# creare-com/pydem

Hardware: AMD Instinct MI355X
Metric: Mcells/s (slope+aspect+UCA+TWI end-to-end) per tile; % HBM roofline (higher is better)
Workload: dtype f64

## Files before the change

### pydem_amd/csrc/pits.hip

```cpp
#include "internal.h"
#include <hipcub/hipcub.hpp>
#include <math.h>
#include <stdlib.h>
#include <algorithm>
#include <vector>

namespace {

__device__ __forceinline__ double np_pairwise_leaf(const double *a, int n)
{
    if (n < 8) {
        double res = 0.;
        for (int i = 0; i < n; i++) res += a[i];
        return res;
    }
    double r0 = a[0], r1 = a[1], r2 = a[2], r3 = a[3], r4 = a[4], r5 = a[5], r6 = a[6], r7 = a[7];
    int i;
    for (i = 8; i < n - (n % 8); i += 8) {
        r0 += a[i]; r1 += a[i + 1]; r2 += a[i + 2]; r3 += a[i + 3];
        r4 += a[i + 4]; r5 += a[i + 5]; r6 += a[i + 6]; r7 += a[i + 7];
    }
    double res = ((r0 + r1) + (r2 + r3)) + ((r4 + r5) + (r6 + r7));
    for (; i < n; i++) res += a[i];
    return res;
// ... 392 lines not shown
        if (gl == 0) {
            if (P.overflow_list && flag[0] == 2) P.overflow_list[atomicAdd(P.overflow_count, 1)] = pit;
            else atomicAdd(&P.out_count[3], 1);
        }
        return;
    }
    if (ndrain < 0) { if (gl == 0) atomicAdd(&P.out_count[1], 1); return; }
    if (gl == 0) finish_pit(P, pit, ipit, jpit, epit, ndrain, dlist, dxy, sv, chunk_base, chunk_left, stk);

}

#ifndef PYDEM_WV_OCC
#define PYDEM_WV_OCC 6
#endif
#ifndef PYDEM_WV_CAP
#define PYDEM_WV_CAP 256
#endif
constexpr int WV_MAXD = 64;
constexpr int LN_W16 = 16;

template <int WW, int CAP, typename PosT>
struct WaveLds {
    static constexpr PosT HOLE = (PosT)~(PosT)0;
    static constexpr PosT PITBIT = (PosT)((PosT)1 << (sizeof(PosT) * 8 - 2));
    uint32_t seen[WW * WW / 32];
    double le[CAP];
    PosT lpos[CAP];
    uint16_t holes[CAP];
    union {
        PosT pq[CAP];
        struct { int32_t dl[WV_MAXD]; double dxy[WV_MAXD], sv[WV_MAXD]; } fin;
    } u;
};

__device__ __forceinline__ double min_f64(double a, double b)
{
    double r;
    asm("v_min_f64 %0, %1, %2" : "=v"(r) : "v"(a), "v"(b));
    return r;
}

template <int CTRL>
__device__ __forceinline__ double dpp_fmin(double v)
{
    const int lo = __double2loint(v), hi = __double2hiint(v);
    const int lo2 = __builtin_amdgcn_update_dpp(0, lo, CTRL, 0xF, 0xF, true);
    const int hi2 = __builtin_amdgcn_update_dpp(0, hi, CTRL, 0xF, 0xF, true);
    return min_f64(v, __hiloint2double(hi2, lo2));
}
#if defined(__HIP_DEVICE_COMPILE__) && !defined(__gfx950__)
#error "wave_min uses the gfx9 DPP row broadcasts (row_bcast:15 / row_bcast:31, removed in gfx10+): this library is built for gfx950 only"
#endif
__device__ __forceinline__ double wave_min(double v)
{
    v = dpp_fmin<0xB1>(v);
    v = dpp_fmin<0x4E>(v);
    v = dpp_fmin<0x141>(v);
    v = dpp_fmin<0x140>(v);
    v = dpp_fmin<0x142>(v);
    v = dpp_fmin<0x143>(v);
    const int lo = __double2loint(v), hi = __double2hiint(v);
    return __hiloint2double(__builtin_amdgcn_readlane(hi, 63), __builtin_amdgcn_readlane(lo, 63));
}
__device__ __forceinline__ void wave_sync()
{
    __builtin_amdgcn_fence(__ATOMIC_SEQ_CST, "wavefront");
    __builtin_amdgcn_wave_barrier();
}

template <int W2, int W2_CAP, typename PosT>
__device__ void solve_pit_wave(const PitParams &P, int32_t pit, int lane, WaveLds<W2, W2_CAP, PosT> &L, int32_t &chunk_base,
                               int32_t &chunk_left, const uint32_t *state = nullptr)
{
    constexpr int W2_SLOTS = W2_CAP / 64;
    constexpr PosT W2_HOLE = WaveLds<W2, W2_CAP, PosT>::HOLE, W2_PITBIT = WaveLds<W2, W2_CAP, PosT>::PITBIT;
    const int n = P.n, m = P.m;
    const int ipit = pit / m, jpit = pit - ipit * m;
    const unsigned long long lt = (1ull << lane) - 1ull;
    int r0 = ipit - W2 / 2, c0 = jpit - W2 / 2;
    if (r0 > n - W2) r0 = n - W2;
    if (c0 > m - W2) c0 = m - W2;
    if (r0 < 0) r0 = 0;
    if (c0 < 0) c0 = 0;
    for (int w = lane; w < W2 * W2 / 32; w += 64) L.seen[w] = 0;
    const double epit = P.elev[pit];
    double epit_border = epit;
    int nb = 0, nh = 0, n_alive = 0;
    bool has_np = false, has_p = false, has_nan = false;
    int over = 0;
    auto expand = [&](int nq) {
        for (int base = 0; base < nq * 8; base += 64) {
            const int idx = base + lane;
            bool isnew = false, out = false;
            double e = 0.0; uint32_t pm = 0; int npos = 0;
            if (idx < nq * 8) {
                const int pos = L.u.pq[idx >> 3], d = idx & 7;
                const int di = d < 3 ? -1 : (d < 5 ? 0 : 1);
                const int dj = d < 3 ? d - 1 : (d == 3 ? -1 : (d == 4 ? 1 : d - 6));
                const int r = pos / W2, c = pos % W2;
                const int ii = r0 + r + di, jj = c0 + c + dj;
                if (ii >= 0 && ii < n && jj >= 0 && jj < m) {
                    const int rr = r + di, cc = c + dj;
                    if (rr < 0 || rr >= W2 || cc < 0 || cc >= W2) out = true;
                    else {
                        npos = rr * W2 + cc;
                        const uint32_t bit = 1u << (npos & 31);
                        const uint32_t old = atomicOr(&L.seen[npos >> 5], bit);
                        if (!(old & bit)) {
                            isnew = true;
                            const int64_t cell = (int64_t)ii * m + jj;
                            e = P.elev[cell]; pm = P.pitmask[cell];
                        }
                    }
                }
            }
            if (__ballot(out)) over = 1;
            const unsigned long long bal = __ballot(isnew);
            const int cnt = __popcll(bal);
            const int fresh = cnt > nh ? cnt - nh : 0;
            if (nb + fresh > W2_CAP) { over = 2; break; }
            if (isnew) {
                const int rk = __popcll(bal & lt);
                const int k = rk < nh ? (int)L.holes[nh - 1 - rk] : nb + (rk - nh);
                L.le[k] = e; L.lpos[k] = (PosT)((PosT)npos | (pm ? W2_PITBIT : (PosT)0));
            }
            if (__ballot(isnew && pm && e < epit)) has_p = true;
            if (__ballot(isnew && !pm && e < epit_border)) has_np = true;
            if (__ballot(isnew && e != e)) has_nan = true;
            nh -= cnt - fresh; nb += fresh; n_alive += cnt;
        }
        wave_sync();
    };
    int it0 = 0, nq0 = 1;
    if (state) {
        it0 = (int)state[0];
        epit_border = __hiloint2double((int)state[3], (int)state[2]);
        int lr0 = ipit - LN_W16 / 2, lc0 = jpit - LN_W16 / 2;
        if (lr0 > n - LN_W16) lr0 = n - LN_W16;
        if (lc0 > m - LN_W16) lc0 = m - LN_W16;
        if (lr0 < 0) lr0 = 0;
        if (lc0 < 0) lc0 = 0;
        const int dpos = (lr0 - r0) * W2 + (lc0 - c0);
        nq0 = 0;
#pragma unroll 1
        for (int j = 0; j < 4; j++) {
            const int cidx = lane + 64 * j;
            const bool in = (state[4 + 2 * j + (lane >> 5)] >> (lane & 31)) & 1u;
            const unsigned long long bal = __ballot(in);
            if (in) {
                const int pos = dpos + (cidx >> 4) * W2 + (cidx & 15);
                atomicOr(&L.seen[pos >> 5], 1u << (pos & 31));
                L.u.pq[nq0 + __popcll(bal & lt)] = (PosT)pos;
            }
            nq0 += __popcll(bal);
        }
    } else if (lane == 0) {
        const int pos = (ipit - r0) * W2 + (jpit - c0);
        L.seen[pos >> 5] = 1u << (pos & 31);
        L.u.pq[0] = (PosT)pos;
    }
    wave_sync();
    expand(nq0);
    if (!state && P.min_border) {
        double mn = INFINITY;
        for (int k = lane; k < nb; k += 64) mn = min_f64(mn, L.le[k]);
        mn = wave_min(mn);
        if (nb) epit_border = mn;
        has_np = false;
    }
    int mode = 0, ndrain = -1, it_used = it0;
    for (int it = it0; it < P.max_iter; it++) {
        if (over) break;
        if (n_alive == 0) break;
        if (has_nan) { if (has_p) mode = 2; break; }
        if (has_np) { mode = 1; break; }
        if (has_p) { mode = 2; break; }
        it_used = it + 1;
        double e[W2_SLOTS];
        double mn = INFINITY;
#pragma unroll
        for (int j = 0; j < W2_SLOTS; j++) {
            const int k = lane + 64 * j;
            e[j] = INFINITY;
            if (j * 64 < nb) {
                if (k < nb) e[j] = L.le[k];
                mn = min_f64(mn, e[j]);
            }
        }
        mn = wave_min(mn);
        int nq = 0;
#pragma unroll
        for (int j = 0; j < W2_SLOTS; j++) {
            if (j * 64 >= nb) break;
            const int k = lane + 64 * j;
            bool match = k < nb && e[j] == mn;
            PosT ps = 0;
            if (match) { ps = L.lpos[k]; match = ps != W2_HOLE; }
            const unsigned long long bal = __ballot(match);
            if (!bal) continue;
            if (match) {
                const int r = nq + __popcll(bal & lt);
                L.u.pq[r] = (PosT)(ps & (PosT)(W2_PITBIT - 1));
                L.holes[nh + r] = (uint16_t)k;
                L.le[k] = INFINITY; L.lpos[k] = W2_HOLE;
            }
            nq += __popcll(bal);
        }
        nh += nq; n_alive -= nq;
        wave_sync();
        expand(nq);
    }
    if (!over && mode) {
        int nd = 0;
        for (int base = 0; base < nb; base += 64) {
            const int k = base + lane;
            bool pred = false;
            int32_t cell = 0;
            if (k < nb && L.lpos[k] != W2_HOLE) {
                const int pos = (int)(L.lpos[k] & (PosT)(W2_PITBIT - 1));
                const bool pm = (L.lpos[k] & W2_PITBIT) != 0;
                const double ev = L.le[k];
                pred = mode == 1 ? (!pm && ev < epit_border) : (pm && ev < epit);
                cell = (int32_t)((int64_t)(r0 + pos / W2) * m + (c0 + pos % W2));
            }
            const unsigned long long bal = __ballot(pred);
            const int rank = nd + __popcll(bal & lt);
            wave_sync();
            if (pred && rank < WV_MAXD) L.u.fin.dl[rank] = cell;
            nd += __popcll(bal);
        }
        if (nd > WV_MAXD) over = 3;
        else {
            wave_sync();
            const int32_t key = lane < nd ? L.u.fin.dl[lane] : INT32_MAX;
            int rank = 0;
            for (int t = 0; t < nd; t++) rank += L.u.fin.dl[t] < key;
            wave_sync();
            if (lane < nd) L.u.fin.dl[rank] = key;
            wave_sync();
            ndrain = nd;
        }
    }
    if (lane == 0 && P.dbg) {
        const int idx = atomicAdd(&P.out_count[6], 1);
        P.dbg[4 * idx] = it_used; P.dbg[4 * idx + 1] = n_alive; P.dbg[4 * idx + 2] = over; P.dbg[4 * idx + 3] = ndrain;
    }
    if (over) {
        if (lane == 0) P.overflow_list[atomicAdd(P.overflow_count, 1)] = pit;
        return;
    }
    if (ndrain < 0) { if (lane == 0) atomicAdd(&P.out_count[1], 1); return; }
    finish_pit_wave(P, pit, ipit, jpit, epit, ndrain, L.u.fin.dl, L.u.fin.dxy, L.u.fin.sv, chunk_base, chunk_left, lane);
}

#include "pits_row.inl"

constexpr int LN_W = 16;
static_assert(LN_W == LN_W16, "hand-over records");
#ifndef PYDEM_LN_B
#define PYDEM_LN_B 32
#endif
constexpr int LN_B = PYDEM_LN_B;
#ifndef PYDEM_LN_T
#define PYDEM_LN_T 64
#endif
constexpr int LN_T = PYDEM_LN_T;

__device__ __forceinline__ double np_pairwise_leaf_strided(const double *a, int stride, int n)
{
    if (n < 8) {
        double res = 0.;
        for (int i = 0; i < n; i++) res += a[i * stride];
        return res;
    }
    double r0 = a[0], r1 = a[stride], r2 = a[2 * stride], r3 = a[3 * stride], r4 = a[4 * stride], r5 = a[5 * stride],
           r6 = a[6 * stride], r7 = a[7 * stride];
    int i;
    for (i = 8; i < n - (n % 8); i += 8) {
        r0 += a[i * stride]; r1 += a[(i + 1) * stride]; r2 += a[(i + 2) * stride]; r3 += a[(i + 3) * stride];
        r4 += a[(i + 4) * stride]; r5 += a[(i + 5) * stride]; r6 += a[(i + 6) * stride]; r7 += a[(i + 7) * stride];
    }
    double res = ((r0 + r1) + (r2 + r3)) + ((r4 + r5) + (r6 + r7));
    for (; i < n; i++) res += a[i * stride];
    return res;
}

__device__ __forceinline__ double np_pairwise_leaf15(const double *__restrict__ a, int n)
{
    double v[15];
#pragma unroll
    for (int k = 0; k < 15; k++) v[k] = a[k < n ? k : (n > 0 ? n - 1 : 0)];
    if (n < 8) {
        double res = 0.;
#pragma unroll
        for (int k = 0; k < 7; k++) if (k < n) res += v[k];
        return res;
    }
    double res = ((v[0] + v[1]) + (v[2] + v[3])) + ((v[4] + v[5]) + (v[6] + v[7]));
#pragma unroll
    for (int k = 8; k < 15; k++) if (k < n) res += v[k];
    return res;
}

constexpr int LN_CHUNK = 256;
constexpr int LN_FIN_BATCH = 32;

__global__ __launch_bounds__(LN_T) void k_pits_lane(PitParams P, const int32_t *__restrict__ pits, const int32_t *npits)
{
    __shared__ double s_e[LN_B * LN_T];
    __shared__ uint8_t s_p[LN_B * LN_T];
    __shared__ uint8_t s_q[LN_B * LN_T];
    __shared__ uint32_t s_seen[8 * LN_T];
    const int tid = threadIdx.x, lane = tid & 63;
    const unsigned long long lt = (1ull << lane) - 1ull;
    const int n = P.n, m = P.m;
    const int32_t np = *npits;
    double *const le = s_e + tid;
    uint8_t *const lp = s_p + tid, *const lq = s_q + tid;
    uint32_t *const seen = s_seen + tid;
    bool running = false, over = false, has_np = false, has_p = false, has_nan = false;
    int pending = 0;
    int32_t pit = 0;
    int r0 = 0, c0 = 0, ipit = 0, jpit = 0, nb = 0, it = 0;
    uint32_t pitbits = 0;
    double epit = 0.0, epit_border = 0.0;
    int32_t chunk_next = 0, chunk_end = 0;
    bool more = true;
    auto discover = [&](int r, int c) {
        const int wa = (r > 0 ? r - 1 : 0) >> 1, wb = (r < LN_W - 1 ? r + 1 : LN_W - 1) >> 1;
        uint32_t va = seen[wa * LN_T], vb = seen[wb * LN_T];
        if (wb == wa) vb = va;
#pragma unroll
        for (int k = 0; k < 8; k++) {
            const int di = k < 3 ? -1 : (k < 5 ? 0 : 1);
            const int dj = k < 3 ? k - 1 : (k == 3 ? -1 : (k == 4 ? 1 : k - 6));
            const int ii = r0 + r + di, jj = c0 + c + dj;
            const int rr = r + di, cc = c + dj;
            if (ii < 0 || ii >= n || jj < 0 || jj >= m) continue;
            if (rr < 0 || rr >= LN_W || cc < 0 || cc >= LN_W) { over = true; continue; }
            const int pos = rr * LN_W + cc;
            const uint32_t bit = 1u << (pos & 31);
            const bool in_a = (pos >> 5) == wa;
            const uint32_t wd = in_a ? va : vb;
            if (wd & bit) continue;
            if (nb == LN_B) { over = true; continue; }
            if (in_a) va |= bit; else vb |= bit;
            if (wb == wa) vb = va;
            lp[nb * LN_T] = (uint8_t)pos;
            nb++;
        }
        seen[wa * LN_T] = va;
        if (wb != wa) seen[wb * LN_T] = vb;
    };
    auto fetch_new = [&](int nb0) {
        constexpr int FB = 8;
        for (int base = nb0; base < nb; base += FB) {
            double e8[FB]; uint8_t pm8[FB];
#pragma unroll
            for (int k = 0; k < FB; k++) {
                e8[k] = 0.0; pm8[k] = 0;
                if (base + k < nb) {
                    const int pos = lp[(base + k) * LN_T];
                    const int64_t cell = (int64_t)(r0 + (pos >> 4)) * m + (c0 + (pos & 15));
                    e8[k] = P.elev[cell]; pm8[k] = P.pitmask[cell];
                }
            }
#pragma unroll
            for (int k = 0; k < FB; k++) {
                const int idx = base + k;
                if (idx >= nb) continue;
                le[idx * LN_T] = e8[k];
                if (e8[k] != e8[k]) has_nan = true;
                if (pm8[k]) { pitbits |= 1u << idx; if (e8[k] < epit) has_p = true; }
                else { pitbits &= ~(1u << idx); if (e8[k] < epit_border) has_np = true; }
            }
        }
    };
    const bool prof = P.prof != nullptr;
    long long acc_a = 0, acc_b = 0, acc_c = 0, acc_g = 0, trips = 0, busy = 0;
    for (;;) {
        long long tk0 = 0, tk1 = 0, tk2 = 0, tkg = 0;
        if (prof) tk0 = clock64();
        const unsigned long long idle = __ballot(!running);
        if (idle && more) {
            if (chunk_next == chunk_end) {
                int32_t b = 0;
                if (lane == 0) b = atomicAdd(P.work_next, LN_CHUNK);
                b = __shfl(b, 0);
                chunk_next = b < np ? b : np;
                chunk_end = b + LN_CHUNK < np ? b + LN_CHUNK : np;
                if (chunk_next >= chunk_end) more = false;
            }
            const int avail = chunk_end - chunk_next, want = __popcll(idle);
            const int rank = __popcll(idle & lt);
            if (!running && rank < avail) {
                pit = pits[chunk_next + rank];
                ipit = pit / m; jpit = pit - ipit * m;
                r0 = ipit - LN_W / 2; c0 = jpit - LN_W / 2;
                if (r0 > n - LN_W) r0 = n - LN_W;
                if (c0 > m - LN_W) c0 = m - LN_W;
                if (r0 < 0) r0 = 0;
                if (c0 < 0) c0 = 0;
#pragma unroll
                for (int w = 0; w < 8; w++) seen[w * LN_T] = 0;
                epit = P.elev[pit];
                epit_border = epit;
                nb = 0; pitbits = 0; it = 0;
                has_np = false; has_p = false; has_nan = false; over = false;
                {
                    const int pos = (ipit - r0) * LN_W + (jpit - c0);
                    seen[(pos >> 5) * LN_T] = 1u << (pos & 31);
                    discover(ipit - r0, jpit - c0);
                    fetch_new(0);
                }
                if (P.min_border) {
                    double mn = INFINITY;
                    for (int k = 0; k < nb; k++) mn = min_f64(mn, le[k * LN_T]);
                    if (nb) epit_border = mn;
                    has_np = false;
                }
                running = true;
            }
            chunk_next += want < avail ? want : avail;
        }
        if (!__ballot(running)) { if (more) continue; break; }
        if (prof) { tk1 = clock64(); busy += __popcll(__ballot(running)); trips++; }
        int nd = 0;
        int status = 0;
        double ssum = 0.0;
        if (running && !pending) {
            if (over) pending = 4;
            else if (it >= P.max_iter || nb == 0) pending = 3;
            else if (has_nan) pending = has_p ? 2 : 3;
            else if (has_np) pending = 1;
            else if (has_p) pending = 2;
            else {
                double mn = INFINITY;
                for (int k0 = 0; k0 < nb; k0 += 8) {
                    double v[8];
#pragma unroll
                    for (int i = 0; i < 8; i++) v[i] = k0 + i < nb ? le[(k0 + i) * LN_T] : INFINITY;
#pragma unroll
                    for (int i = 0; i < 8; i++) mn = min_f64(mn, v[i]);
                }
                uint32_t eq = 0;
                for (int k0 = 0; k0 < nb; k0 += 8) {
                    double v[8];
#pragma unroll
                    for (int i = 0; i < 8; i++) v[i] = k0 + i < nb ? le[(k0 + i) * LN_T] : INFINITY;
#pragma unroll
                    for (int i = 0; i < 8; i++) if (k0 + i < nb && v[i] == mn) eq |= 1u << (k0 + i);
                }
                int nq = 0;
                while (eq) {
                    const int k = 31 - __clz((int)eq);
                    eq &= ~(1u << k);
                    lq[nq * LN_T] = lp[k * LN_T]; nq++;
                    nb--;
                    if (k != nb) {
                        le[k * LN_T] = le[nb * LN_T]; lp[k * LN_T] = lp[nb * LN_T];
                        pitbits = (pitbits & ~(1u << k)) | (((pitbits >> nb) & 1u) << k);
                    }
                }
                const int nb0 = nb;
                for (int j = 0; j < nq; j++) { const int pos = lq[j * LN_T]; discover(pos >> 4, pos & 15); }
                fetch_new(nb0);
                it++;
            }
        }
        const unsigned long long waiting = __ballot(pending != 0), growing = __ballot(running && !pending);
        if (prof) { tkg = clock64(); acc_g += tkg - tk1; }
        if (!(__popcll(waiting) >= LN_FIN_BATCH || (waiting && !growing))) continue;
        if (pending) {
            const int mode = pending <= 2 ? pending : 0;
            status = pending == 4 ? 3 : 2;
            if (mode) {
                uint32_t mt = 0;
                for (int k0 = 0; k0 < nb; k0 += 8) {
                    double v[8];
#pragma unroll
                    for (int i = 0; i < 8; i++) v[i] = k0 + i < nb ? le[(k0 + i) * LN_T] : INFINITY;
#pragma unroll
                    for (int i = 0; i < 8; i++) {
                        const bool isp = (pitbits >> (k0 + i)) & 1u;
                        if (k0 + i < nb && (mode == 1 ? (!isp && v[i] < epit_border) : (isp && v[i] < epit))) mt |= 1u << (k0 + i);
                    }
                }
                while (mt) {
                    const int k = __ffs((int)mt) - 1;
                    mt &= mt - 1u;
                    if (k != nd) {
                        const double ek = le[k * LN_T], en = le[nd * LN_T];
                        const uint8_t pk = lp[k * LN_T], pn = lp[nd * LN_T];
                        const uint32_t bk = (pitbits >> k) & 1u, bn = (pitbits >> nd) & 1u;
                        le[k * LN_T] = en; lp[k * LN_T] = pn; le[nd * LN_T] = ek; lp[nd * LN_T] = pk;
                        pitbits = (pitbits & ~((1u << k) | (1u << nd))) | (bn << k) | (bk << nd);
                    }
                    nd++;
                }
                for (int a = 1; a < nd; a++) {
                    const double ea = le[a * LN_T]; const uint8_t pa = lp[a * LN_T]; const uint32_t ba = (pitbits >> a) & 1u;
                    int b = a - 1;
                    while (b >= 0 && lp[b * LN_T] > pa) {
                        le[(b + 1) * LN_T] = le[b * LN_T]; lp[(b + 1) * LN_T] = lp[b * LN_T];
                        pitbits = (pitbits & ~(1u << (b + 1))) | (((pitbits >> b) & 1u) << (b + 1));
                        b--;
                    }
                    le[(b + 1) * LN_T] = ea; lp[(b + 1) * LN_T] = pa;
                    pitbits = (pitbits & ~(1u << (b + 1))) | (ba << (b + 1));
                }
                const int ndX = n - 1;
                const bool xy = !isnan(P.max_dist_XY) && P.max_dist_XY != 0;
                int keep = 0;
                for (int t = 0; t < nd; t++) {
                    const int pos = lp[t * LN_T];
                    const int idr = r0 + (pos >> 4), jdr = c0 + (pos & 15);
                    if (P.max_dist) {
                        const int di = ipit - idr, dj = jpit - jdr;
                        if (!(sqrt((double)(di * di + dj * dj)) <= (double)P.max_dist)) continue;
                    }
                    const int a = ipit < idr ? ipit : idr, b = ipit < idr ? idr : ipit;
                    double dxm;
                    if (ipit == idr) dxm = P.dX[ipit < ndX - 1 ? ipit : ndX - 1];
                    else dxm = np_pairwise_leaf15(P.dX + a, b - a) / (double)(b - a);
                    const double dx = dxm * (double)(jpit - jdr);
                    const double dy = np_pairwise_leaf15(P.dY + a, b - a);
                    const double d = sqrt(dx * dx + dy * dy);
                    if (xy && !(d <= P.max_dist_XY)) continue;
                    le[keep * LN_T] = pit_drop(P, epit, le[t * LN_T]) / d;
                    lp[keep * LN_T] = (uint8_t)pos;
                    keep++;
                }
                nd = keep;
                if (nd > 0) {
                    ssum = np_pairwise_leaf_strided(le, LN_T, nd);
                    P.mag[pit] = ssum / (double)nd;
                    P.flats[pit] = 0;
                    status = 1;
                }
            }
            running = false; pending = 0;
        }
        if (prof) { tk2 = clock64(); acc_a += tk1 - tk0; acc_b += tk2 - tkg; }
        if (!__ballot(status != 0)) continue;
        int incl = nd;
        for (int off = 1; off < 64; off <<= 1) { const int o = __shfl_up(incl, off); if (lane >= off) incl += o; }
        const int tot = __shfl(incl, 63);
        int32_t wbase = 0;
        if (lane == 0 && tot) wbase = atomicAdd(&P.out_count[0], tot);
        wbase = __shfl(wbase, 0);
        if (tot) {
            if ((int64_t)wbase + tot <= P.out_cap) {
                const int32_t o = wbase + incl - nd;
                for (int t = 0; t < nd; t++) {
                    const int pos = lp[t * LN_T];
                    P.out_src[o + t] = pit;
                    P.out_dst[o + t] = (int32_t)((int64_t)(r0 + (pos >> 4)) * m + (c0 + (pos & 15)));
                    P.out_w[o + t] = le[t * LN_T] / ssum;
                }
            } else if (lane == 0) atomicAdd(&P.out_count[3], 1);
        }
        const unsigned long long b_un = __ballot(status == 2), b_ov = __ballot(status == 3);
        if (lane == 0 && b_un) atomicAdd(&P.out_count[1], __popcll(b_un));
        if (b_ov) {
            int32_t obase = 0;
            if (lane == 0) obase = atomicAdd(&P.out_count[4], __popcll(b_ov));
            obase = __shfl(obase, 0);
            if (status == 3) {
                const int32_t slot = obase + __popcll(b_ov & lt);
                P.lane_overflow[slot] = pit;
                if (P.lane_state) {
                for (int k = 0; k < nb; k++) { const int pos = lp[k * LN_T]; seen[(pos >> 5) * LN_T] &= ~(1u << (pos & 31)); }
                uint32_t *rec = P.lane_state + (size_t)slot * 12;
                rec[0] = (uint32_t)it; rec[1] = 0;
                rec[2] = (uint32_t)__double2loint(epit_border); rec[3] = (uint32_t)__double2hiint(epit_border);
#pragma unroll
                for (int w = 0; w < 8; w++) rec[4 + w] = seen[w * LN_T];
                }
            }
        }
        if (prof) acc_c += clock64() - tk2;
    }
    if (prof && lane == 0) {
        atomicAdd(P.prof + 0, (unsigned long long)acc_a); atomicAdd(P.prof + 1, (unsigned long long)acc_b);
        atomicAdd(P.prof + 2, (unsigned long long)acc_c); atomicAdd(P.prof + 3, (unsigned long long)busy);
        atomicAdd(P.prof + 4, (unsigned long long)trips); atomicAdd(P.prof + 5, (unsigned long long)acc_g);
    }
}

constexpr int W_LARGE = 640, MAXD_LARGE = 2048;

template <int CAP, int OCC>
__global__ __launch_bounds__(256, OCC) void k_pits_wave(PitParams P, const int32_t *__restrict__ pits, const int32_t *npits)
{
    __shared__ WaveLds<128, CAP, uint16_t> s_l[4];
    const int wave = threadIdx.x >> 6, lane = threadIdx.x & 63;
    const int32_t np = *npits;
    int32_t chunk_base = 0, chunk_left = 0;
    for (;;) {
        int32_t q = 0;
        if (lane == 0) q = atomicAdd(P.work_next, 1);
        q = __shfl(q, 0);
        if (q >= np) break;
        if (P.wave_index) q = P.wave_index[q];
        solve_pit_wave(P, pits[q], lane, s_l[wave], chunk_base, chunk_left, P.lane_state ? P.lane_state + (size_t)q * 12 : nullptr);
        wave_sync();
    }
}

__global__ __launch_bounds__(64) void k_pits_wave_big(PitParams P, const int32_t *__restrict__ pits, const int32_t *npits)
{
    __shared__ WaveLds<256, 2048, uint32_t> s_l;
    const int lane = threadIdx.x;
    const int32_t np = *npits;
    int32_t chunk_base = 0, chunk_left = 0;
    for (int32_t q = blockIdx.x; q < np; q += gridDim.x) {
        solve_pit_wave(P, pits[q], lane, s_l, chunk_base, chunk_left);
        wave_sync();
    }
}

#ifndef PYDEM_BLOCK_NT
#define PYDEM_BLOCK_NT 512
#endif
constexpr int BLOCK_NT = PYDEM_BLOCK_NT;
__global__ __launch_bounds__(BLOCK_NT) void k_pits_block(PitParams P, const int32_t *__restrict__ pits, const int32_t *npits,
                                                    int32_t *g_dl, double *g_dxy, double *g_sv, int maxd)
{
    constexpr int WORDS = W_LARGE * W_LARGE / 32;
    extern __shared__ __attribute__((aligned(16))) uint32_t dyn[];
    __shared__ double redd[BLOCK_NT / 64];
    __shared__ int redi[BLOCK_NT / 64];
    __shared__ int flag[4];
    __shared__ PwFrame stk[16];
    int32_t chunk_base = 0, chunk_left = 0;
    const int32_t np = *npits;
    for (int32_t q = blockIdx.x; q < np; q += gridDim.x) {
        solve_pit<BLOCK_NT, W_LARGE>(P, pits[q], threadIdx.x, dyn, dyn + WORDS, dyn + 2 * WORDS,
                                     g_dl + (size_t)blockIdx.x * maxd, g_dxy + (size_t)blockIdx.x * maxd,
                                     g_sv + (size_t)blockIdx.x * maxd, redd, redi, flag, chunk_base, chunk_left, stk, maxd);
        __syncthreads();
    }
}

__global__ void k_pitmask(const uint8_t *__restrict__ flats, const double *__restrict__ elev, int64_t NN, uint8_t *pitmask)
{
    const int64_t nvec = NN >> 4, stride = (int64_t)gridDim.x * blockDim.x, t0 = (int64_t)blockIdx.x * blockDim.x + threadIdx.x;
    for (int64_t v = t0; v < nvec; v += stride) {
        const uint4 f4 = reinterpret_cast<const uint4 *>(flats)[v];
        const uint32_t fw[4] = {f4.x, f4.y, f4.z, f4.w};
        uint32_t pw[4];
#pragma unroll
        for (int q = 0; q < 4; q++) {
            uint32_t p = 0;
            if (fw[q])
#pragma unroll
                for (int b = 0; b < 4; b++)
                    if (((fw[q] >> (8 * b)) & 0xFFu) && elev[v * 16 + q * 4 + b] > 0) p |= 1u << (8 * b);
            pw[q] = p;
        }
        reinterpret_cast<uint4 *>(pitmask)[v] = make_uint4(pw[0], pw[1], pw[2], pw[3]);
    }
    for (int64_t c = (nvec << 4) + t0; c < NN; c += stride) pitmask[c] = flats[c] && (elev[c] > 0);
}

__global__ __launch_bounds__(256) void k_compact_mask(const uint8_t *__restrict__ mask, int64_t NN,
                                                       int32_t *__restrict__ list, int32_t *__restrict__ count)
{
    __shared__ int32_t wave_tot[4][4];
    __shared__ int32_t blk_base;
    const int lane = threadIdx.x & 63, wave = threadIdx.x >> 6;
    for (int64_t base = (int64_t)blockIdx.x * 65536; base < NN; base += (int64_t)gridDim.x * 65536) {
        unsigned long long bits[4];
        int32_t mine[4], incl[4];
#pragma unroll
        for (int j = 0; j < 4; j++) {
            const int64_t c0 = base + j * 16384 + (int64_t)threadIdx.x * 64;
            bits[j] = 0;
            if (c0 + 64 <= NN) {
                uint4 v[4];
#pragma unroll
                for (int q = 0; q < 4; q++) v[q] = *reinterpret_cast<const uint4 *>(mask + c0 + 16 * q);
#pragma unroll
                for (int q = 0; q < 4; q++) {
                    const uint32_t w[4] = {v[q].x, v[q].y, v[q].z, v[q].w};
#pragma unroll
                    for (int k = 0; k < 16; k++)
                        bits[j] |= (unsigned long long)(((w[k >> 2] >> (8 * (k & 3))) & 0xffu) ? 1u : 0u) << (16 * q + k);
                }
            } else {
                for (int k = 0; k < 64; k++)
                    if (c0 + k < NN && mask[c0 + k]) bits[j] |= 1ull << k;
            }
            mine[j] = __popcll(bits[j]);
            incl[j] = mine[j];
#pragma unroll
            for (int off = 1; off < 64; off <<= 1) {
                const int32_t o = __shfl_up(incl[j], off);
                if (lane >= off) incl[j] += o;
            }
            if (lane == 63) wave_tot[j][wave] = incl[j];
        }
        __syncthreads();
        if (threadIdx.x == 0) {
            int32_t tot = 0;
            for (int j = 0; j < 4; j++) for (int k = 0; k < 4; k++) tot += wave_tot[j][k];
            blk_base = tot ? atomicAdd(count, tot) : 0;
        }
        __syncthreads();
        int32_t off = blk_base;
#pragma unroll
        for (int j = 0; j < 4; j++) {
            int32_t o = off + incl[j] - mine[j];
            for (int k = 0; k < wave; k++) o += wave_tot[j][k];
            const int64_t c0 = base + j * 16384 + (int64_t)threadIdx.x * 64;
            unsigned long long b = bits[j];
            while (b) {
                const int k = __ffsll((long long)b) - 1;
                b &= b - 1;
                list[o++] = (int32_t)(c0 + k);
            }
            off += wave_tot[j][0] + wave_tot[j][1] + wave_tot[j][2] + wave_tot[j][3];
        }
        __syncthreads();
    }
}

__global__ __launch_bounds__(256) void k_pit_keys(const int32_t *__restrict__ src, const int32_t *__restrict__ dst, const double *__restrict__ w,
                                                  const double *__restrict__ elev, int32_t ne, uint64_t *key_out, uint64_t *key_in, int32_t *idx,
                                                  int32_t *count, int kb)
{
    constexpr int PER = 4;
    __shared__ int32_t wave_tot[4];
    __shared__ int32_t blk_base;
    const int lane = threadIdx.x & 63, wave = threadIdx.x >> 6;
    for (int64_t base = (int64_t)blockIdx.x * (256 * PER); base < ne; base += (int64_t)gridDim.x * (256 * PER)) {
        uint32_t keep = 0;
        int32_t sv[PER], dv[PER];
#pragma unroll
        for (int j = 0; j < PER; j++) {
            const int64_t e = base + j * 256 + threadIdx.x;
            sv[j] = -1; dv[j] = 0;
            if (e < ne) { sv[j] = src[e]; dv[j] = dst[e]; }
        }
#pragma unroll
        for (int j = 0; j < PER; j++) {
            const int64_t e = base + j * 256 + threadIdx.x;
            if (sv[j] >= 0) {
                const double we = w[e];
                if (!isnan(we) && we > 1e-8 && elev[dv[j]] <= elev[sv[j]]) keep |= 1u << j;
            }
        }
        const int32_t mine = __popc(keep);
        int32_t incl = mine;
#pragma unroll
        for (int off = 1; off < 64; off <<= 1) { const int32_t o = __shfl_up(incl, off); if (lane >= off) incl += o; }
        if (lane == 63) wave_tot[wave] = incl;
        __syncthreads();
        if (threadIdx.x == 0) {
            const int32_t tot = wave_tot[0] + wave_tot[1] + wave_tot[2] + wave_tot[3];
            blk_base = tot ? atomicAdd(count, tot) : 0;
        }
        __syncthreads();
        int32_t o = blk_base + incl - mine;
        for (int k = 0; k < wave; k++) o += wave_tot[k];
#pragma unroll
        for (int j = 0; j < PER; j++)
            if (keep & (1u << j)) {
                key_out[o] = ((uint64_t)(uint32_t)sv[j] << kb) | (uint32_t)dv[j];
                key_in[o] = ((uint64_t)(uint32_t)dv[j] << kb) | (uint32_t)sv[j];
                idx[o] = (int32_t)(base + j * 256 + threadIdx.x);
                o++;
            }
        __syncthreads();
    }
}

__global__ void k_pit_gather(const uint64_t *__restrict__ keys, const int32_t *__restrict__ idx, const double *__restrict__ w,
                             int32_t ne, int swap, int32_t *a, int32_t *b, double *wo, int32_t *dup, int kb)
{
    for (int32_t e = blockIdx.x * blockDim.x + threadIdx.x; e < ne; e += gridDim.x * blockDim.x) {
        const uint64_t k = keys[e];
        if (dup && e > 0 && keys[e - 1] == k) atomicAdd(dup, 1);
        const int32_t hi = (int32_t)(k >> kb), lo = (int32_t)(k & ((1ull << kb) - 1ull));
        a[e] = swap ? lo : hi;
        b[e] = swap ? hi : lo;
        wo[e] = w[idx[e]];
    }
}

template <typename T>
int dev_realloc(pydem_tile *t, T **p, size_t count)
{
    if (*p) { plane_give(t->device, *p); *p = nullptr; }
    return tile_alloc(t, p, count);
}

}

int stage_pits(pydem_tile *t, const pydem_options *opt)
{
    const int n = (int)t->n, m = (int)t->m;
    if (opt->drain_pits_max_iter > 300) {
        pydem_set_error("drain_pits_max_iter > 300 is not supported by the device window (got %d)", opt->drain_pits_max_iter);
        return -2;
    }
    HIP_TRY(hipEventRecord(t->ev[4], t->stream));
    PYDEM_TRY(tile_alloc(t, &t->flat0, (size_t)t->NN));
    PYDEM_TRY(tile_alloc(t, &t->flatlist, (size_t)t->NN));
    PYDEM_TRY(tile_alloc(t, &t->labels, (size_t)t->NN));
    PYDEM_TRY(tile_alloc(t, &t->queue[0], (size_t)t->NN));
    int32_t *cnt = t->counters + 40;
    HIP_TRY(hipMemsetAsync(cnt, 0, 16 * sizeof(int32_t), t->stream));
    const int big = (int)(cdiv(t->NN, 256) < 8192 ? cdiv(t->NN, 256) : 8192);
    hipLaunchKernelGGL(k_pitmask, dim3(big), dim3(256), 0, t->stream, t->flats, t->elev, t->NN, t->flat0);
    hipLaunchKernelGGL(k_compact_mask, dim3((unsigned)(cdiv(t->NN, 4096) < 4096 ? cdiv(t->NN, 4096) : 4096)), dim3(256), 0,
                       t->stream, t->flat0, t->NN, t->flatlist, cnt);
    HIP_TRY(hipMemcpyAsync(t->h_counters, cnt, sizeof(int32_t), hipMemcpyDeviceToHost, t->stream));
    HIP_TRY(hipStreamSynchronize(t->stream));
    const int32_t npits = t->h_counters[0];
    t->tm.n_pit_edges = 0; t->tm.n_pits_undrained = 0;
    t->tm.n_pits = npits; t->tm.n_pits_row = 0; t->tm.n_pits_wave = 0; t->tm.n_pits_big = 0;
    t->pits.n_edges = 0;
    if (npits == 0) { t->tm.pits_ms = 0; return 0; }

    int64_t cap = (int64_t)npits * 2 + 16384 * 4 * OUT_CHUNK + 1024;
    for (int attempt = 0;; attempt++) {
        if (t->pits.raw_cap < cap) {
            PYDEM_TRY(dev_realloc(t, &t->pits.raw_src, (size_t)cap));
            PYDEM_TRY(dev_realloc(t, &t->pits.raw_dst, (size_t)cap));
            PYDEM_TRY(dev_realloc(t, &t->pits.raw_w, (size_t)cap));
            t->pits.raw_cap = cap;
        }
        HIP_TRY(hipMemsetAsync(cnt + 1, 0, 8 * sizeof(int32_t), t->stream));
        PitParams P;
        P.dbg = nullptr; P.prof = nullptr;
        const char *dbg_env = getenv("PYDEM_PITS_DEBUG");
        if (dbg_env && atoi(dbg_env) == 3) { HIP_TRY(hipMalloc(&P.prof, 128)); HIP_TRY(hipMemsetAsync(P.prof, 0, 128, t->stream)); }
        if (dbg_env && atoi(dbg_env) >= 2) HIP_TRY(hipMalloc(&P.dbg, (size_t)npits * 16));
        HIP_TRY(hipMemsetAsync(t->pits.raw_src, 0xFF, (size_t)t->pits.raw_cap * 4, t->stream));
        P.elev = t->elev; P.pitmask = t->flat0; P.dX = t->dX; P.dY = t->dY; P.mag = t->mag; P.flats = t->flats;
        P.n = n; P.m = m; P.max_iter = opt->drain_pits_max_iter; P.max_dist = opt->drain_pits_max_dist;
        P.min_border = opt->drain_pits_min_border; P.max_dist_XY = opt->drain_pits_max_dist_XY;
        P.elev_f32 = t->elev_f32 ? 1 : 0;
        P.out_src = t->pits.raw_src; P.out_dst = t->pits.raw_dst; P.out_w = t->pits.raw_w;
        P.out_count = cnt + 1; P.out_cap = (int32_t)(t->pits.raw_cap < INT32_MAX ? t->pits.raw_cap : INT32_MAX);
// ... 210 lines not shown
```

Before: 5458.

## Prefetch next pit and its neighbours, double-buffer work chunks, single-pass min scan

Each lane now prefetches its next pit's id, elevation and 8-neighbour elevation/pitmask values while its current pit is still running. Work chunks are double-buffered, with pit ids held in registers and distributed via shuffles. The goal is to hide the global-load latency that used to stall lane restarts. The neighbour fetch becomes branch-free by clamping indices, and the min search merges two passes into one. In exchange the kernel uses more registers, which could lower occupancy, and it issues redundant clamped loads.

```diff
diff --git a/pydem_amd/csrc/pits.hip b/pydem_amd/csrc/pits.hip
--- a/pydem_amd/csrc/pits.hip
+++ b/pydem_amd/csrc/pits.hip
@@ -718,7 +718,11 @@
     return res;
 }
 
-constexpr int LN_CHUNK = 256;
+#ifndef PYDEM_LN_CHUNK
+#define PYDEM_LN_CHUNK 256
+#endif
+constexpr int LN_CHUNK = PYDEM_LN_CHUNK;
+static_assert(LN_CHUNK % 64 == 0 && LN_CHUNK >= 64, "chunk ids in registers");
 constexpr int LN_FIN_BATCH = 32;
 
 __global__ __launch_bounds__(LN_T) void k_pits_lane(PitParams P, const int32_t *__restrict__ pits, const int32_t *npits)
@@ -740,8 +744,14 @@
     int r0 = 0, c0 = 0, ipit = 0, jpit = 0, nb = 0, it = 0;
     uint32_t pitbits = 0;
     double epit = 0.0, epit_border = 0.0;
-    int32_t chunk_next = 0, chunk_end = 0;
+    int32_t chunk_lo = 0, chunk_next = 0, chunk_end = 0, nlo = 0, nend = 0;
+    int32_t ids[LN_CHUNK / 64] = {}, nids[LN_CHUNK / 64] = {};
+    bool nready = false;
     bool more = true;
+    bool nx_have = false;
+    int32_t nx_pit = 0;
+    double nx_epit = 0.0, nx_e[8] = {};
+    uint8_t nx_pm[8] = {};
     auto discover = [&](int r, int c) {
         const int wa = (r > 0 ? r - 1 : 0) >> 1, wb = (r < LN_W - 1 ? r + 1 : LN_W - 1) >> 1;
         uint32_t va = seen[wa * LN_T], vb = seen[wb * LN_T];
@@ -771,76 +781,122 @@
     auto fetch_new = [&](int nb0) {
         constexpr int FB = 8;
         for (int base = nb0; base < nb; base += FB) {
-            double e8[FB]; uint8_t pm8[FB];
+            double e8[FB]; uint8_t pm8[FB]; int ix8[FB];
 #pragma unroll
             for (int k = 0; k < FB; k++) {
-                e8[k] = 0.0; pm8[k] = 0;
-                if (base + k < nb) {
-                    const int pos = lp[(base + k) * LN_T];
-                    const int64_t cell = (int64_t)(r0 + (pos >> 4)) * m + (c0 + (pos & 15));
-                    e8[k] = P.elev[cell]; pm8[k] = P.pitmask[cell];
-                }
+                ix8[k] = base + k < nb ? base + k : nb - 1;
+                const int pos = lp[ix8[k] * LN_T];
+                const int64_t cell = (int64_t)(r0 + (pos >> 4)) * m + (c0 + (pos & 15));
+                e8[k] = P.elev[cell]; pm8[k] = P.pitmask[cell];
             }
 #pragma unroll
             for (int k = 0; k < FB; k++) {
-                const int idx = base + k;
-                if (idx >= nb) continue;
+                const int idx = ix8[k];
                 le[idx * LN_T] = e8[k];
-                if (e8[k] != e8[k]) has_nan = true;
-                if (pm8[k]) { pitbits |= 1u << idx; if (e8[k] < epit) has_p = true; }
-                else { pitbits &= ~(1u << idx); if (e8[k] < epit_border) has_np = true; }
-            }
-        }
+                const bool isp = pm8[k] != 0, below = e8[k] < (isp ? epit : epit_border);
+                has_nan = has_nan | (e8[k] != e8[k]);
+                pitbits = (pitbits & ~(1u << idx)) | ((uint32_t)isp << idx);
+                has_p = has_p | (isp & below); has_np = has_np | (!isp & below);
+            }
+        }
+    };
+    auto next_chunk = [&]() {
+        int32_t b = 0;
+        if (lane == 0) b = atomicAdd(P.work_next, LN_CHUNK);
+        b = __builtin_amdgcn_readfirstlane(b);
+        nlo = b < np ? b : np;
+        nend = b + LN_CHUNK < np ? b + LN_CHUNK : np;
+#pragma unroll
+        for (int j = 0; j < LN_CHUNK / 64; j++) {
+            const int32_t q = nlo + 64 * j + lane;
+            nids[j] = q < nend ? pits[q] : 0;
+        }
+        nready = true;
     };
     const bool prof = P.prof != nullptr;
     long long acc_a = 0, acc_b = 0, acc_c = 0, acc_g = 0, trips = 0, busy = 0;
     for (;;) {
         long long tk0 = 0, tk1 = 0, tk2 = 0, tkg = 0;
         if (prof) tk0 = clock64();
-        const unsigned long long idle = __ballot(!running);
-        if (idle && more) {
-            if (chunk_next == chunk_end) {
-                int32_t b = 0;
-                if (lane == 0) b = atomicAdd(P.work_next, LN_CHUNK);
-                b = __shfl(b, 0);
-                chunk_next = b < np ? b : np;
-                chunk_end = b + LN_CHUNK < np ? b + LN_CHUNK : np;
-                if (chunk_next >= chunk_end) more = false;
-            }
-            const int avail = chunk_end - chunk_next, want = __popcll(idle);
-            const int rank = __popcll(idle & lt);
-            if (!running && rank < avail) {
-                pit = pits[chunk_next + rank];
-                ipit = pit / m; jpit = pit - ipit * m;
-                r0 = ipit - LN_W / 2; c0 = jpit - LN_W / 2;
-                if (r0 > n - LN_W) r0 = n - LN_W;
-                if (c0 > m - LN_W) c0 = m - LN_W;
-                if (r0 < 0) r0 = 0;
-                if (c0 < 0) c0 = 0;
-#pragma unroll
-                for (int w = 0; w < 8; w++) seen[w * LN_T] = 0;
-                epit = P.elev[pit];
-                epit_border = epit;
-                nb = 0; pitbits = 0; it = 0;
-                has_np = false; has_p = false; has_nan = false; over = false;
-                {
-                    const int pos = (ipit - r0) * LN_W + (jpit - c0);
-                    seen[(pos >> 5) * LN_T] = 1u << (pos & 31);
-                    discover(ipit - r0, jpit - c0);
-                    fetch_new(0);
-                }
-                if (P.min_border) {
-                    double mn = INFINITY;
-                    for (int k = 0; k < nb; k++) mn = min_f64(mn, le[k * LN_T]);
-                    if (nb) epit_border = mn;
-                    has_np = false;
-                }
-                running = true;
+        if (!running && nx_have) {
+            pit = nx_pit;
+            ipit = pit / m; jpit = pit - ipit * m;
+            r0 = ipit - LN_W / 2; c0 = jpit - LN_W / 2;
+            if (r0 > n - LN_W) r0 = n - LN_W;
+            if (c0 > m - LN_W) c0 = m - LN_W;
+            if (r0 < 0) r0 = 0;
+            if (c0 < 0) c0 = 0;
+#pragma unroll
+            for (int w = 0; w < 8; w++) seen[w * LN_T] = 0;
+            epit = nx_epit;
+            epit_border = epit;
+            nb = 0; pitbits = 0; it = 0;
+            has_np = false; has_p = false; has_nan = false; over = false;
+            {
+                const int pos = (ipit - r0) * LN_W + (jpit - c0);
+                seen[(pos >> 5) * LN_T] = 1u << (pos & 31);
+                discover(ipit - r0, jpit - c0);
+                int idx = 0;
+#pragma unroll
+                for (int k = 0; k < 8; k++) {
+                    const int di = k < 3 ? -1 : (k < 5 ? 0 : 1);
+                    const int dj = k < 3 ? k - 1 : (k == 3 ? -1 : (k == 4 ? 1 : k - 6));
+                    const int ii = ipit + di, jj = jpit + dj;
+                    if (ii < 0 || ii >= n || jj < 0 || jj >= m) continue;
+                    const double e = nx_e[k];
+                    le[idx * LN_T] = e;
+                    if (e != e) has_nan = true;
+                    const bool isp = nx_pm[k] != 0, below = e < epit;
+                    pitbits |= (uint32_t)isp << idx;
+                    has_p = has_p | (isp & below); has_np = has_np | (!isp & below);
+                    idx++;
+                }
+            }
+            if (P.min_border) {
+                double mn = INFINITY;
+                for (int k = 0; k < nb; k++) mn = min_f64(mn, le[k * LN_T]);
+                if (nb) epit_border = mn;
+                has_np = false;
+            }
+            running = true; nx_have = false;
+        }
+        if (more && chunk_next == chunk_end) {
+            if (!nready) next_chunk();
+#pragma unroll
+            for (int j = 0; j < LN_CHUNK / 64; j++) ids[j] = nids[j];
+            chunk_lo = chunk_next = nlo; chunk_end = nend;
+            nready = false;
+            if (chunk_next >= chunk_end) more = false;
+        }
+        const unsigned long long empty = __ballot(!nx_have);
+        if (empty && more) {
+            const int avail = chunk_end - chunk_next, want = __popcll(empty);
+            const int rank = __popcll(empty & lt);
+            const int o = chunk_next - chunk_lo + rank;
+            int32_t id = 0;
+#pragma unroll
+            for (int j = 0; j < LN_CHUNK / 64; j++) { const int32_t v = __shfl(ids[j], o & 63); if ((o >> 6) == j) id = v; }
+            if (!nx_have && rank < avail) {
+                nx_pit = id;
+                const int pi = id / m, pj = id - pi * m;
+                nx_epit = P.elev[id];
+#pragma unroll
+                for (int k = 0; k < 8; k++) {
+                    const int di = k < 3 ? -1 : (k < 5 ? 0 : 1);
+                    const int dj = k < 3 ? k - 1 : (k == 3 ? -1 : (k == 4 ? 1 : k - 6));
+                    const int ii = pi + di, jj = pj + dj;
+                    nx_e[k] = 0.0; nx_pm[k] = 0;
+                    if (ii < 0 || ii >= n || jj < 0 || jj >= m) continue;
+                    const int64_t cell = (int64_t)ii * m + jj;
+                    nx_e[k] = P.elev[cell]; nx_pm[k] = P.pitmask[cell];
+                }
+                nx_have = true;
             }
             chunk_next += want < avail ? want : avail;
         }
-        if (!__ballot(running)) { if (more) continue; break; }
-        if (prof) { tk1 = clock64(); busy += __popcll(__ballot(running)); trips++; }
+        if (more && !nready && chunk_end - chunk_next <= LN_CHUNK / 2) next_chunk();
+        if (!__ballot(running)) { if (more || __ballot(nx_have)) continue; break; }
+        if (prof) { tk1 = clock64(); acc_a += tk1 - tk0; busy += __popcll(__ballot(running)); trips++; }
         int nd = 0;
         int status = 0;
         double ssum = 0.0;
@@ -852,20 +908,17 @@
             else if (has_p) pending = 2;
             else {
                 double mn = INFINITY;
-                for (int k0 = 0; k0 < nb; k0 += 8) {
-                    double v[8];
-#pragma unroll
-                    for (int i = 0; i < 8; i++) v[i] = k0 + i < nb ? le[(k0 + i) * LN_T] : INFINITY;
-#pragma unroll
-                    for (int i = 0; i < 8; i++) mn = min_f64(mn, v[i]);
-                }
                 uint32_t eq = 0;
                 for (int k0 = 0; k0 < nb; k0 += 8) {
                     double v[8];
 #pragma unroll
                     for (int i = 0; i < 8; i++) v[i] = k0 + i < nb ? le[(k0 + i) * LN_T] : INFINITY;
 #pragma unroll
-                    for (int i = 0; i < 8; i++) if (k0 + i < nb && v[i] == mn) eq |= 1u << (k0 + i);
+                    for (int i = 0; i < 8; i++) {
+                        if (k0 + i >= nb) continue;
+                        if (v[i] < mn) { mn = v[i]; eq = 1u << (k0 + i); }
+                        else if (v[i] == mn) eq |= 1u << (k0 + i);
+                    }
                 }
                 int nq = 0;
                 while (eq) {
@@ -957,7 +1010,7 @@
             }
             running = false; pending = 0;
         }
-        if (prof) { tk2 = clock64(); acc_a += tk1 - tk0; acc_b += tk2 - tkg; }
+        if (prof) { tk2 = clock64(); acc_b += tk2 - tkg; }
         if (!__ballot(status != 0)) continue;
         int incl = nd;
         for (int off = 1; off < 64; off <<= 1) { const int o = __shfl_up(incl, off); if (lane >= off) incl += o; }
```

After: 5531, median of 6. 1.01x the previous value.
